# nikvaessen/w2v2-speaker

Hardware: AMD Instinct MI355X
Metric: utterances/sec (w2v2-base + mean+std + AAM-softmax training step, 3 s clips) (higher is better)
Workload: dtype f16; 1 GPU; wav2vec2-base + AAM-softmax(5994), mean+std pooling, 3 s synthetic audio, bs=66 per GPU, CNN frozen, fwd+bwd+all-reduce+Adam (BASELINE configs[1]); global_batch=66, samples_per_utt=48000, parallelism=dp1, regularisation=True

## Files before the change

### include/w2v2_hip.h

```cpp
#ifndef W2V2_HIP_H
#define W2V2_HIP_H

#include <stddef.h>
#include <stdint.h>

#ifdef __cplusplus
extern "C" {
#endif

#define W2V2_F32 0
#define W2V2_BF16 1
#define W2V2_F16 2

int w2v2_version(void);
const char* w2v2_last_error(void);

typedef struct {
  const void* ptr;
  int64_t ld;
  int64_t seg_len, seg_stride;
  int64_t stride0, stride1;
  int32_t trans;
  int32_t _pad;
} w2v2_operand;
// ... 25 lines not shown
  const float* row_scale;
  const float* col_scale;
  float alpha;
  int32_t split_k;
  int32_t accumulate;
  int32_t _pad;
  int32_t k_ext, n_ext_from;
  int64_t b_lo_offset;
} w2v2_gemm_desc;

int w2v2_gemm(const w2v2_gemm_desc* d, void* stream);
int w2v2_gemm_timed(const w2v2_gemm_desc* d, void* stream, int slot);
int w2v2_timer_read(int first_slot, int n, float* ms_out);
int w2v2_gemm_kernel_of(const w2v2_gemm_desc* d);
int w2v2_tune_gemm_kernel(int family);
int w2v2_tune_gemm_debug(int bits);
int w2v2_tune_gemm_f32_tile(int tile);
int w2v2_tune_gemm_ring_debug(int bits);
int w2v2_gemm_f32_last_kernel(void);

typedef struct {
  const void* dY; int64_t ld_dy;
  const void* X;  int64_t ld_x;
  float* dW;      int64_t ld_dw;
  float* dbias;
  int32_t n_out, n_in;
} w2v2_wgrad_problem;
int w2v2_wgrad_grouped(const w2v2_wgrad_problem* problems, int n, int tokens, int tokens_padded,
                       int dtype , void* stream);
int w2v2_wgrad_kernel_of(const w2v2_wgrad_problem* problems, int n);
// ... 358 lines not shown
```

### w2v2_speaker_amd/_lib.py

```python
from __future__ import annotations

import ctypes as C
import os

from . import _build

F32, BF16, F16 = 0, 1, 2
EPI_NONE, EPI_BIAS, EPI_BIAS_GELU, EPI_GELU_BWD, EPI_ADD, EPI_SCALE_RC, EPI_BIAS_GELU_GRAD, EPI_MUL = range(8)
OPTIM_ADAM, OPTIM_SGD = 0, 1

c_i32, c_i64, c_u64, c_f32, c_f64, c_vp = C.c_int32, C.c_int64, C.c_uint64, C.c_float, C.c_double, C.c_void_p


class Operand(C.Structure):
    _fields_ = [("ptr", c_vp), ("ld", c_i64), ("seg_len", c_i64), ("seg_stride", c_i64),
                ("stride0", c_i64), ("stride1", c_i64), ("trans", c_i32), ("_pad", c_i32)]


class GemmDesc(C.Structure):
    _fields_ = [("M", c_i32), ("N", c_i32), ("K", c_i32), ("batch", c_i32), ("batch_inner", c_i32),
                ("dtype_ab", c_i32), ("dtype_c", c_i32), ("epilogue", c_i32),
                ("A", Operand), ("B", Operand),
                ("C", c_vp), ("ldc", c_i64), ("c_stride0", c_i64), ("c_stride1", c_i64),
                ("aux", c_vp), ("ldaux", c_i64), ("aux_stride0", c_i64), ("aux_stride1", c_i64),
# ... 7 lines not shown


class WgradProblem(C.Structure):
    _fields_ = [("dY", c_vp), ("ld_dy", c_i64), ("X", c_vp), ("ld_x", c_i64), ("dW", c_vp), ("ld_dw", c_i64),
                ("dbias", c_vp), ("n_out", c_i32), ("n_in", c_i32)]


_SIGS = {
    "w2v2_version": (c_i32, []),
    "w2v2_last_error": (C.c_char_p, []),
    "w2v2_gemm": (c_i32, [C.POINTER(GemmDesc), c_vp]),
    "w2v2_gemm_kernel_of": (c_i32, [c_vp]),
    "w2v2_gemm_timed": (c_i32, [C.POINTER(GemmDesc), c_vp, c_i32]),
    "w2v2_timer_read": (c_i32, [c_i32, c_i32, c_vp]),
    "w2v2_tune_gemm_kernel": (c_i32, [c_i32]),
    "w2v2_tune_gemm_debug": (c_i32, [c_i32]),
    "w2v2_tune_gemm_f32_tile": (c_i32, [c_i32]),
    "w2v2_tune_gemm_ring_debug": (c_i32, [c_i32]),
    "w2v2_gemm_f32_last_kernel": (c_i32, []),
    "w2v2_zero_ranges": (c_i32, [c_vp, c_vp, c_i32, c_i32, c_vp]),
    "w2v2_mean": (c_i32, [c_vp, c_vp, c_i32, c_vp]),
    "w2v2_wgrad_grouped": (c_i32, [C.POINTER(WgradProblem), c_i32, c_i32, c_i32, c_i32, c_vp]),
    "w2v2_wgrad_kernel_of": (c_i32, [C.POINTER(WgradProblem), c_i32]),
    "w2v2_tune_wgrad_kernel": (c_i32, [c_i32]),
    "w2v2_conv0_workspace_floats": (c_i32, [c_i32, c_i32, c_i32, c_i32]),
    "w2v2_conv0_stats": (c_i32, [c_vp, c_vp, c_vp, c_vp, c_i32, c_i32, c_i32, c_i32, c_i32, c_f32, c_vp]),
    "w2v2_conv0_stats_mfma": (c_i32, [c_vp, c_vp, c_vp, c_vp, c_i32, c_i32, c_i32, c_i32, c_i32, c_f32, c_vp]),
    "w2v2_conv0_stats_len": (c_i32, [c_vp, c_vp, c_vp, c_vp, c_vp, c_i32, c_i32, c_i32, c_i32, c_i32, c_f32, c_vp]),
    "w2v2_conv0_stats_mfma_len": (c_i32, [c_vp, c_vp, c_vp, c_vp, c_vp, c_i32, c_i32, c_i32, c_i32, c_i32, c_f32,
                                          c_vp]),
# ... 210 lines not shown
```

### w2v2_speaker_amd/csrc/common.h

```cpp
#pragma once
#include <hip/hip_runtime.h>
#include <hip/hip_ext.h>
#include <stdint.h>
#include <stdio.h>
#include <math.h>
#include <type_traits>
#include <utility>

#include "../../include/w2v2_hip.h"

extern thread_local char g_w2v2_err[512];
#define W2V2_FAIL(...)                                   \
  do {                                                   \
    snprintf(g_w2v2_err, sizeof(g_w2v2_err), __VA_ARGS__); \
    return -1;                                           \
  } while (0)
#define W2V2_CHECK_LAUNCH(name)                                                       \
  do {                                                                                \
    hipError_t e__ = hipGetLastError();                                               \
    if (e__ != hipSuccess) W2V2_FAIL("%s: launch failed: %s", name, hipGetErrorString(e__)); \
  } while (0)
#define W2V2_REQUIRE(cond, ...) \
  do {                          \
    if (!(cond)) W2V2_FAIL(__VA_ARGS__); \
// ... 29 lines not shown
    }
  }
  hipLaunchKernelGGL(KERNEL, grid, block, lds, st, args...);
  return 0;
}

struct W2v2Switches {
  bool no_glds;
  bool glds3;
  bool tile256;
  bool persistent;
  int g3n;
  bool defer;
  bool wt_stores;
  bool late_dma;
  int reserve_cus;
  bool f32_no_dma;
  bool wgrad_ring;
  bool wgrad_ring4;
  bool wgrad_phased;
};
const W2v2Switches& w2v2_switches();
int w2v2_device_cus();

__device__ __forceinline__ void w2v2_dma16(const void* src, uint32_t lds_addr) {
  asm volatile("s_mov_b32 m0, %0\n\ts_nop 0\n\tglobal_load_lds_dwordx4 %1, off" ::"s"(lds_addr), "v"(src) : "memory", "m0");
}
__device__ __forceinline__ void w2v2_dma16(const void* src, void* lds) {
  w2v2_dma16(src, __builtin_amdgcn_readfirstlane((uint32_t)(uintptr_t)(__attribute__((address_space(3))) char*)lds));
}
// ... 376 lines not shown
```

### w2v2_speaker_amd/csrc/gemm.hip

```cpp
#include "gemm_common.h"

template <int R, bool TRANS>
struct Stager {
  static constexpr int NV = TRANS ? 4 : (R / 32);
  uint4 v[NV];

  __device__ __forceinline__ void load(const OpDev& o, const bf16_t* __restrict__ base, int r0,
                                       int rbound, int k0, int kend, int tid,
                                       const int64_t* __restrict__ rowoff) {
    if constexpr (!TRANS) {
#pragma unroll
      for (int j = 0; j < NV; ++j) {
        const int c = tid + 256 * j;
        const int row = c >> 3, kc = c & 7;
        const int k = k0 + kc * 8;
        uint4 val = make_uint4(0, 0, 0, 0);
        if (r0 + row < rbound && k < kend) {
          const bf16_t* p = base + rowoff[j] + k;
          if (o.vec_ok && k + 8 <= kend) {
            val = *reinterpret_cast<const uint4*>(p);
          } else {
            bf16_t t[8];
#pragma unroll
            for (int e = 0; e < 8; ++e) t[e] = (k + e < kend) ? p[e] : (bf16_t)0;
// ... 264 lines not shown
}

const W2v2Switches& w2v2_switches() {
  static const W2v2Switches sw = [] {
    W2v2Switches s;
    auto env_int = [](const char* name, int dflt) { const char* e = getenv(name); return e ? atoi(e) : dflt; };
    auto env_on = [](const char* name, bool dflt) { const char* e = getenv(name); return e ? e[0] != '0' : dflt; };
    s.no_glds = getenv("W2V2_NO_GLDS") != nullptr;
    s.glds3 = getenv("W2V2_NO_GLDS3") == nullptr;
    s.tile256 = getenv("W2V2_NO_GEMM_PH") == nullptr;
    s.persistent = getenv("W2V2_G3_NONPERSISTENT") == nullptr;
    s.g3n = env_int("W2V2_G3N", 512);
    s.defer = getenv("W2V2_NO_DEFER") == nullptr;
    s.wt_stores = env_on("W2V2_EPI_WT", true);
    s.late_dma = env_on("W2V2_PH_LATE", false);
    s.reserve_cus = env_int("W2V2_RESERVE_CUS", 0);
    s.f32_no_dma = env_on("W2V2_F32_NO_DMA", false);
    s.wgrad_ring = getenv("W2V2_WGRAD_V1") == nullptr;
    s.wgrad_ring4 = getenv("W2V2_NO_WGRAD4") == nullptr;
    s.wgrad_phased = getenv("W2V2_NO_WGRAD_PH") == nullptr;
    return s;
  }();
  return sw;
}

int w2v2_device_cus() {
  static const int ncu = [] {
    int dev = 0, v = 0;
    (void)hipGetDevice(&dev);
    return (hipDeviceGetAttribute(&v, hipDeviceAttributeMultiprocessorCount, dev) == hipSuccess && v > 0) ? v : 256;
  }();
  return ncu;
}
int w2v2_gemm_device_cus() {
  const int ncu = w2v2_device_cus(), r = w2v2_switches().reserve_cus;
  return (r > 0 && r < ncu) ? ncu - r : ncu;
}

static int g_w2v2_force = 0;
extern "C" int w2v2_tune_gemm_kernel(int family) {
  const int old = g_w2v2_force;
  if (family == 0 || family == 1 || family == 2 || family == 4) g_w2v2_force = family;
  return old;
}

struct GemmRoute {
  int family;
  bool narrow;
  dim3 grid;
  int f32_rows;
};

static bool aligned16(const void* p) { return (reinterpret_cast<uintptr_t>(p) & 15) == 0; }

static int gemm_route(const w2v2_gemm_desc* d, int force, GemmArgs& a, GemmRoute& r) {
  W2V2_REQUIRE(d != nullptr, "w2v2_gemm: null descriptor");
  W2V2_REQUIRE(d->M > 0 && d->N > 0 && d->K >= 0 && d->batch > 0, "w2v2_gemm: bad shape M=%d N=%d K=%d batch=%d",
               d->M, d->N, d->K, d->batch);
  W2V2_REQUIRE(d->A.ptr && d->B.ptr && d->C, "w2v2_gemm: null operand");
  W2V2_REQUIRE(d->dtype_ab == W2V2_F32 || d->dtype_ab == W2V2_BF16 || d->dtype_ab == W2V2_F16,
               "w2v2_gemm: bad dtype_ab %d", d->dtype_ab);
  W2V2_REQUIRE(d->dtype_c == W2V2_F32 || d->dtype_c == d->dtype_ab, "w2v2_gemm: dtype_c %d must be f32 or dtype_ab (%d)",
               d->dtype_c, d->dtype_ab);
  W2V2_REQUIRE(d->epilogue >= 0 && d->epilogue <= W2V2_EPI_MUL, "w2v2_gemm: bad epilogue %d", d->epilogue);
  const int split = d->split_k > 1 ? d->split_k : 1;
  const int atomic = (split > 1 || d->accumulate) ? 1 : 0;
  if (atomic) {
    W2V2_REQUIRE(d->dtype_c == W2V2_F32, "w2v2_gemm: split_k/accumulate need an f32 C");
    W2V2_REQUIRE(d->epilogue == W2V2_EPI_NONE || (split == 1) || d->epilogue == W2V2_EPI_BIAS,
                 "w2v2_gemm: split_k supports EPI_NONE/EPI_BIAS only");
// ... 25 lines not shown
  a.C = d->C; a.ldc = d->ldc; a.c_s0 = d->c_stride0; a.c_s1 = d->c_stride1;
  a.aux = d->aux; a.ldaux = d->ldaux; a.aux_s0 = d->aux_stride0; a.aux_s1 = d->aux_stride1;
  a.bias = d->bias; a.bias_s1 = d->bias_stride1;
  a.row_scale = d->row_scale; a.col_scale = d->col_scale;
  a.alpha = d->alpha;
  a.k_ext = d->k_ext; a.n_ext_from = d->n_ext_from; a.b_lo_off = d->b_lo_offset;
  a.defer_ok = 0;
  a.wt_stores = 1;
  a.late_dma = 0;
  a.xcd_tiles = 0;
  a.dbg_bits = 0;
  const int cal = d->dtype_c == W2V2_F32 ? 4 : 8;
  a.c_vec_ok = aligned16(d->C) && (d->ldc % cal == 0) && (d->c_stride0 % cal == 0) && (d->c_stride1 % cal == 0);
  a.aux_vec_ok = d->aux && aligned16(d->aux) && (d->ldaux % cal == 0) && (d->aux_stride0 % cal == 0) &&
                 (d->aux_stride1 % cal == 0);
  r.family = 0; r.narrow = false; r.grid = dim3(1); r.f32_rows = 0;

  const int bk = f32 ? 32 : 64;
  a.k_per_split = (int)(cdiv(cdiv(d->K, split), bk) * bk);
  if (a.k_per_split == 0) a.k_per_split = bk;
  if (f32) {
    r.f32_rows = w2v2_gemm_f32_dma_rows(a, d->M, d->N, d->K, split, d->batch);
    r.family = r.f32_rows > 0 ? 10 : 9;
    return 0;
  }

  const W2v2Switches& sw = w2v2_switches();
  const int64_t ncu = w2v2_gemm_device_cus();
  const bool glds = !a.A.trans && !a.B.trans && a.A.vec_ok && a.B.vec_ok && (d->K % 64 == 0) && d->K >= 64 && !sw.no_glds;
  r.narrow = d->N <= 64 || (glds && cdiv(d->M, 128) * cdiv(d->N, 128) * split * d->batch * 2 <= ncu);
  a.tiles_m = (int)cdiv(d->M, 128); a.tiles_n = (int)cdiv(d->N, r.narrow ? 64 : 128);
// ... 11 lines not shown
    phased = force == 4 && phased_ok;
  } else {
    ring = ring_ok && (d->k_ext != 0 || (d->N >= sw.g3n && d->M >= 1024 && sw.glds3));
    phased = false;
    if (ring && phased_ok && d->N >= 512 && sw.tile256) {
      const int64_t t4 = cdiv(d->M, 256) * cdiv(d->N, 256), t3 = cdiv(d->M, 256) * cdiv(d->N, 128);
      const double fill4 = (double)t4 / (double)(cdiv(t4, ncu) * ncu), fill3 = (double)t3 / (double)(cdiv(t3, ncu) * ncu);
      phased = fill4 * 1.25 >= fill3 && t4 * 2 >= ncu && (double)d->N / (double)(cdiv(d->N, 256) * 256) >= 0.9;
    }
  }
  if (d->k_ext != 0)
    W2V2_REQUIRE(ring && d->k_ext == d->K && d->n_ext_from >= 0 && d->n_ext_from % 128 == 0 && d->b_lo_offset % 8 == 0,
                 "w2v2_gemm: two-term weights (k_ext) need k_ext == K, n_ext_from %% 128 == 0 and K-contiguous 16-byte "
                 "aligned operands with K %% 64 == 0 (M=%d N=%d K=%d)", d->M, d->N, d->K);
  r.family = phased ? 4 : ring ? 2 : glds ? 1 : 3;
  a.wt_stores = sw.wt_stores;
  a.late_dma = sw.late_dma;
  if (r.family == 2)
    a.defer_ok = sw.defer && d->dtype_c != W2V2_F32 && lines_ok(a) && (d->N % 128 == 0) &&
                 d->epilogue != W2V2_EPI_BIAS_GELU && d->epilogue != W2V2_EPI_BIAS_GELU_GRAD;
  return 0;
}

extern "C" int w2v2_gemm_kernel_of(const w2v2_gemm_desc* d) {
  GemmArgs a;
  GemmRoute r;
  return gemm_route(d, g_w2v2_force, a, r) != 0 ? -1 : r.family;
}

template <typename TE, int FM, int FN, typename TC>
static int launch_glds(const GemmArgs& a, dim3 grid, hipStream_t st) {
  constexpr size_t lds = (size_t)2 * (32 * FM + 32 * FN) * 64 * sizeof(bf16_t);
  return w2v2_launch_lds<&gemm16_dma_128_kernel<TE, FM, FN, TC>>("gemm16_dma_128_kernel", grid, dim3(256), lds, st, a);
}

template <typename TE, int FM, int FN, typename TC>
static int launch_regstage(const GemmArgs& a, dim3 grid, hipStream_t st) {
  constexpr size_t lds = (size_t)2 * (32 * FM + 32 * FN) * 64 * sizeof(bf16_t);
#define W2V2_LAUNCH(TA_, TB_) \
  return w2v2_launch_lds<&gemm16_regstage_kernel<TE, FM, FN, TA_, TB_, TC>>("gemm16_regstage_kernel", grid, dim3(256), lds, st, a)
  if (!a.A.trans && !a.B.trans) W2V2_LAUNCH(false, false);
  else if (!a.A.trans && a.B.trans) W2V2_LAUNCH(false, true);
  else if (a.A.trans && !a.B.trans) W2V2_LAUNCH(true, false);
  else W2V2_LAUNCH(true, true);
#undef W2V2_LAUNCH
}

template <typename TE, typename TC>
static int launch_128(const GemmArgs& a, const GemmRoute& r, hipStream_t st) {
  if (r.family == 1) return r.narrow ? launch_glds<TE, 4, 2, TC>(a, r.grid, st) : launch_glds<TE, 4, 4, TC>(a, r.grid, st);
  return r.narrow ? launch_regstage<TE, 4, 2, TC>(a, r.grid, st) : launch_regstage<TE, 4, 4, TC>(a, r.grid, st);
}

extern "C" int w2v2_gemm(const w2v2_gemm_desc* d, void* stream) {
  GemmArgs a;
  GemmRoute r;
  if (gemm_route(d, g_w2v2_force, a, r) != 0) return -1;
  hipStream_t st = as_stream(stream);
  const bool c32 = d->dtype_c == W2V2_F32;
  int rc;
  switch (r.family) {
    case 4: rc = w2v2_launch_phased_256x256(a, d->dtype_ab, d->dtype_c, d->M, d->N, d->batch, st); break;
    case 2: rc = w2v2_launch_ring_256x128(a, d->dtype_ab, d->dtype_c, d->M, d->N, d->batch, w2v2_switches().persistent, st); break;
    case 9: case 10: rc = w2v2_launch_gemm_f32(a, d->M, d->N, d->K, a.split_k, d->batch, r.f32_rows, st); break;
    default:
      if (d->dtype_ab == W2V2_BF16) rc = c32 ? launch_128<bf16_t, float>(a, r, st) : launch_128<bf16_t, bf16_t>(a, r, st);
      else rc = c32 ? launch_128<f16_t, float>(a, r, st) : launch_128<f16_t, f16_t>(a, r, st);
      break;
  }
  if (rc != 0) return rc;
  W2V2_CHECK_LAUNCH("w2v2_gemm");
  return 0;
}

#include <vector>
W2v2PendingTimer& w2v2_pending_timer() {
  static thread_local W2v2PendingTimer t = {nullptr, nullptr, false};
// ... 32 lines not shown
```

### w2v2_speaker_amd/csrc/gemm_common.h

```cpp
#pragma once
#include "common.h"
#include <hip/hip_ext.h>
#include <type_traits>
#include <stdlib.h>

struct OpDev {
  const void* ptr;
  int64_t ld, seg_len, seg_stride;
  int trans;
  int vec_ok;
};

struct GemmArgs {
  int M, N, K;
  int epilogue, split_k, atomic;
  int tiles_m, tiles_n;
  int k_per_split;
  OpDev A, B;
  int64_t a_s0, a_s1, b_s0, b_s1;
  int batch_inner;
  void* C;
  int64_t ldc, c_s0, c_s1;
  void* aux;
  int64_t ldaux, aux_s0, aux_s1;
// ... 205 lines not shown

__device__ __forceinline__ void load_col8(const GemmArgs& g, const float* __restrict__ bias, int n, float (&cv)[8]) {
  const float* src = (g.epilogue == W2V2_EPI_SCALE_RC) ? g.col_scale : bias;
#pragma unroll
  for (int e = 0; e < 8; ++e) cv[e] = 0.f;
  if (src == nullptr || n >= g.N) return;
  if (n + 8 <= g.N && ((reinterpret_cast<uintptr_t>(src + n) & 15) == 0)) {
    const float4 a = *reinterpret_cast<const float4*>(src + n), b = *reinterpret_cast<const float4*>(src + n + 4);
    cv[0] = a.x; cv[1] = a.y; cv[2] = a.z; cv[3] = a.w; cv[4] = b.x; cv[5] = b.y; cv[6] = b.z; cv[7] = b.w;
  } else {
#pragma unroll
    for (int e = 0; e < 8; ++e) if (n + e < g.N) cv[e] = src[n + e];
  }
}

template <typename TC, int EPI, int FM, int I0, bool DEFER = false, int NR = 4>
__device__ __forceinline__ void epilogue_direct4(const GemmArgs& g, TC* __restrict__ Cz, TC* __restrict__ auxz,
                                                 f32x4 (&acc)[FM][4], int m, int n, const float (&cv0)[8],
                                                 const float (&cv1)[8], uint4 (&pend)[8]) {
  float ax[NR][16];
  if constexpr (EPI == W2V2_EPI_GELU_BWD || EPI == W2V2_EPI_ADD || EPI == W2V2_EPI_MUL) {
#pragma unroll
    for (int i = 0; i < NR; ++i) {
      const int mi = m + 16 * (I0 + i);
#pragma unroll
      for (int e = 0; e < 16; ++e) ax[i][e] = 0.f;
      if (mi < g.M) {
        const TC* ap = auxz + (int64_t)mi * g.ldaux + n;
#pragma unroll
        for (int h = 0; h < 2; ++h) {
          if (n + 8 * h + 8 <= g.N && g.aux_vec_ok) {
            Vec8<TC> t;
            t.load(ap + 8 * h);
#pragma unroll
            for (int e = 0; e < 8; ++e) ax[i][8 * h + e] = t.v[e];
          } else {
#pragma unroll
            for (int e = 0; e < 8; ++e) if (n + 8 * h + e < g.N) ax[i][8 * h + e] = to_f32<TC>(ap[8 * h + e]);
          }
        }
      }
    }
  }
#pragma unroll
  for (int i = 0; i < NR; ++i) {
    const int mi = m + 16 * (I0 + i);
    if (mi >= g.M) continue;
#pragma unroll
    for (int h = 0; h < 2; ++h) {
      if (n + 8 * h >= g.N) continue;
      float v[8];
#pragma unroll
      for (int e = 0; e < 8; ++e) v[e] = acc[I0 + i][2 * h + (e >> 2)][e & 3];
      float a8[8];
#pragma unroll
      for (int e = 0; e < 8; ++e) a8[e] = (EPI == W2V2_EPI_GELU_BWD || EPI == W2V2_EPI_ADD || EPI == W2V2_EPI_MUL) ? ax[i][8 * h + e] : 0.f;
      if constexpr (DEFER && FM == 4)
        epilogue_row8_impl<TC, EPI, true>(g, Cz, auxz, mi, n + 8 * h, v, h ? cv1 : cv0, a8, true, &pend[i * 2 + h]);
      else
        epilogue_row8_impl<TC, EPI>(g, Cz, auxz, mi, n + 8 * h, v, h ? cv1 : cv0, a8, true);
    }
  }
}
template <typename TC, int EPI, int FM, int NR = 4>
__device__ __forceinline__ void epilogue_direct(const GemmArgs& g, TC* __restrict__ Cz, TC* __restrict__ auxz,
                                                f32x4 (&acc)[FM][4], int m, int n, const float (&cv0)[8],
                                                const float (&cv1)[8]) {
  if (n >= g.N) return;
  uint4 unused[8];
  if constexpr (NR == 4) {
    epilogue_direct4<TC, EPI, FM, 0>(g, Cz, auxz, acc, m, n, cv0, cv1, unused);
    if constexpr (FM > 4) epilogue_direct4<TC, EPI, FM, 4>(g, Cz, auxz, acc, m, n, cv0, cv1, unused);
  } else {
    static_assert(NR == 2 && FM == 8, "two-row batches are wired for the 128-row wave tiles");
    epilogue_direct4<TC, EPI, FM, 0, false, 2>(g, Cz, auxz, acc, m, n, cv0, cv1, unused);
    epilogue_direct4<TC, EPI, FM, 2, false, 2>(g, Cz, auxz, acc, m, n, cv0, cv1, unused);
    epilogue_direct4<TC, EPI, FM, 4, false, 2>(g, Cz, auxz, acc, m, n, cv0, cv1, unused);
    epilogue_direct4<TC, EPI, FM, 6, false, 2>(g, Cz, auxz, acc, m, n, cv0, cv1, unused);
  }
}

__host__ __device__ __forceinline__ bool lines_ok(const GemmArgs& g) {
  return g.c_vec_ok && !g.atomic && (g.N & 63) == 0 && (g.aux == nullptr || g.aux_vec_ok);
}

template <typename TC, int EPI, int FM, bool DEFER = false>
__device__ __forceinline__ void epilogue_lines(const GemmArgs& g, TC* __restrict__ Cz, TC* __restrict__ auxz,
                                               f32x4 (&acc)[FM][4], int mw, int nc, int lane, const float (&cv0)[8],
                                               const float (&cv1)[8], uint4* __restrict__ pend) {
  static_assert(sizeof(TC) == 2, "16-bit outputs only");
  constexpr bool READS_AUX = EPI == W2V2_EPI_GELU_BWD || EPI == W2V2_EPI_ADD || EPI == W2V2_EPI_MUL;
  constexpr bool WRITES_AUX = EPI == W2V2_EPI_BIAS_GELU || EPI == W2V2_EPI_BIAS_GELU_GRAD;
  if constexpr (!DEFER) {
    if (nc >= g.N) return;
  }
  const bool wt = g.wt_stores != 0;
  auto st16 = [wt](TC* p, uint4 v) {
    if (wt) store16_wt(p, v); else *reinterpret_cast<uint4*>(p) = v;
  };
  const int c = lane & 15;
  const bool lo = c < 8;
  const int ra = mw + (c & 7);
  const int ncs = nc + (lo ? 0 : 8);
  const int mo = mw + c;
#pragma unroll
  for (int i0 = 0; i0 < FM; i0 += 4) {
    uint4 la[4], lb[4];
    if constexpr (READS_AUX) {
#pragma unroll
      for (int i = 0; i < 4; ++i) {
        const int r = ra + 16 * (i0 + i);
        la[i] = lb[i] = make_uint4(0, 0, 0, 0);
        if (r < g.M) la[i] = *reinterpret_cast<const uint4*>(auxz + (int64_t)r * g.ldaux + ncs);
        if (r + 8 < g.M) lb[i] = *reinterpret_cast<const uint4*>(auxz + (int64_t)(r + 8) * g.ldaux + ncs);
      }
    }
#pragma unroll
    for (int i = 0; i < 4; ++i) {
      float ax[16];
      if constexpr (READS_AUX) {
        uint4 a0, a1;
        lines_to_halves(lo, la[i], lb[i], a0, a1);
        unpack8<TC>(a0, ax);
        unpack8<TC>(a1, ax + 8);
      }
      float rs = 1.0f;
      if constexpr (EPI == W2V2_EPI_SCALE_RC) rs = (mo + 16 * (i0 + i) < g.M) ? g.row_scale[mo + 16 * (i0 + i)] : 0.f;
      float v[16], pre[16];
#pragma unroll
      for (int e = 0; e < 16; ++e) {
        float x = acc[i0 + i][e >> 2][e & 3] * g.alpha;
        const float cve = e < 8 ? cv0[e] : cv1[e - 8];
        if constexpr (EPI == W2V2_EPI_BIAS) x += cve;
// ... 116 lines not shown
__device__ __forceinline__ void ring_tile_srcs(const GemmArgs& g, const bf16_t* Ab, const bf16_t* Bb, int m0, int n0,
                                               int wave, int lane, const bf16_t** ap, const bf16_t** bp) {
  const int c8 = lane & 7, r8 = lane >> 3;
  int ca[4], cb[2];
#pragma unroll
  for (int j = 0; j < 4; ++j) ca[j] = (c8 ^ swz((wave * 4 + j) * 8 + r8)) << 3;
#pragma unroll
  for (int j = 0; j < 2; ++j) cb[j] = (c8 ^ swz_b((wave * 2 + j) * 8 + r8)) << 3;
  tile_ptrs<4>(g.A, Ab, m0, 256, g.M, wave * 32 + r8, 8, ca, ap);
  tile_ptrs<2>(g.B, Bb, n0, 128, g.N, wave * 16 + r8, 8, cb, bp);
}

int w2v2_gemm_device_cus();
int w2v2_launch_ring_256x128(const GemmArgs& a, int dtype_ab, int dtype_c, int M, int N, int batch, bool persistent,
                             hipStream_t st);
int w2v2_launch_phased_256x256(const GemmArgs& a, int dtype_ab, int dtype_c, int M, int N, int batch, hipStream_t st);
int w2v2_launch_gemm_f32(GemmArgs a, int M, int N, int K, int split, int batch, int dma_rows, hipStream_t st);
int w2v2_gemm_f32_dma_rows(const GemmArgs& a, int M, int N, int K, int split, int batch);
int w2v2_launch_gemm_f32_dma(const GemmArgs& a, int M, int N, int split, int batch, int fi, int nst, hipStream_t st);
bool w2v2_gemm_f32_dma_has_dbg(const GemmArgs& a, int fi);
```

### w2v2_speaker_amd/csrc/gemm_phased.hip

```cpp
#include "gemm_common.h"

template <typename TE, typename TC, int DBG = 0>
__global__ __launch_bounds__(512) void gemm16_phased_256x256_kernel(const GemmArgs g) {
  constexpr int BM = 256, BN = 256, BK = 64, FM = 8, FN = 4;
  constexpr int BUF = (BM + BN) * BK;
  extern __shared__ __attribute__((aligned(16))) char smem_raw[];
  bf16_t* smem = reinterpret_cast<bf16_t*>(smem_raw);

  const int tid = threadIdx.x;
  const int lane = tid & 63;
  const int wave = __builtin_amdgcn_readfirstlane(tid >> 6);
  const int wr = wave >> 2, wc = wave & 3;
  const int ntile = g.tiles_m * g.tiles_n;
  const int G = gridDim.x;
  const int z = blockIdx.z;
  const int z0 = z / g.batch_inner, z1 = z - z0 * g.batch_inner;
  const int nk = g.K >> 6;
  const bf16_t* Ab = reinterpret_cast<const bf16_t*>(g.A.ptr) + z0 * g.a_s0 + z1 * g.a_s1;
  const bf16_t* Bb = reinterpret_cast<const bf16_t*>(g.B.ptr) + z0 * g.b_s0 + z1 * g.b_s1;
  const int c8 = lane & 7, r8 = lane >> 3;
  const int frow = lane & 15, fk = lane >> 4;
  const int sw = swz(frow);
  const int la0 = (wr * 128 + frow) * 64 + ((fk ^ sw) << 3);
  const int la1 = (wr * 128 + frow) * 64 + (((4 + fk) ^ sw) << 3);
  const int brow = (frow >> 2) * 16 + (frow & 3);
  const int lb0 = BM * 64 + (wc * 64 + brow) * 64 + ((fk ^ sw) << 3);
  const int lb1 = BM * 64 + (wc * 64 + brow) * 64 + (((4 + fk) ^ sw) << 3);
  auto piece_row = [&](int q, int j) -> int {
    const int p = wave * 2 + j;
    if (q == 0) return (p < 8 ? p * 8 : 128 + (p - 8) * 8);
    if (q == 3) return (p < 8 ? p * 8 : 128 + (p - 8) * 8) + 64;
    return p * 16 + (q == 2 ? 8 : 0);
  };

#pragma unroll 1
  for (int t0 = 0; t0 < ntile; t0 += G) {
    const int nchunk = min(G, ntile - t0);
    if ((int)blockIdx.x >= nchunk) break;
    const int tile = t0 + xcd_remap(blockIdx.x, nchunk);
    const int tm = tile / g.tiles_n, tn = tile - tm * g.tiles_n;
    const int m0 = tm * BM, n0 = tn * BN;
    int soff[4][2];
// ... 2 lines not shown
      const bool isa = q == 0 || q == 3;
      int col[2];
      const bf16_t* ptr[2];
#pragma unroll
      for (int j = 0; j < 2; ++j) {
        const int row = piece_row(q, j) + r8;
        col[j] = (c8 ^ (isa ? swz(row) : swz_b(row))) << 3;
      }
      if (isa) tile_ptrs<2>(g.A, Ab, m0, BM, g.M, piece_row(q, 0) + r8, 8, col, ptr);
      else tile_ptrs<2>(g.B, Bb, n0, BN, g.N, piece_row(q, 0) + r8, 16, col, ptr);
#pragma unroll
      for (int j = 0; j < 2; ++j) soff[q][j] = (int)(ptr[j] - (isa ? Ab : Bb));
    }
    auto issue = [&](int q, int kt) {
      const bool isa = q == 0 || q == 3;
      bf16_t* base = smem + (kt & 1) * BUF + (isa ? 0 : BM * 64);
#pragma unroll
      for (int j = 0; j < 2; ++j)
        w2v2_dma16(((isa ? Ab : Bb) + (soff[q][j] + kt * 64)), (base + piece_row(q, j) * 64));
    };
    f32x4 acc[FM][FN];
#pragma unroll
    for (int i = 0; i < FM; ++i)
#pragma unroll
      for (int j = 0; j < FN; ++j) acc[i][j] = f32x4{0.f, 0.f, 0.f, 0.f};

    issue(0, 0); issue(1, 0); issue(2, 0); issue(3, 0);
    if (nk > 1) { issue(0, 1); issue(1, 1); }
    w2v2_vmcnt0_visible();
    __builtin_amdgcn_s_barrier();
    if (wr == 1) __builtin_amdgcn_s_barrier();
// ... 4 lines not shown
    if constexpr (NO_READ) {
#pragma unroll
      for (int j = 0; j < 2; ++j)
#pragma unroll
        for (int kk = 0; kk < 2; ++kk) {
          b0[j][kk] = *reinterpret_cast<const frag8_t*>(smem + (kk ? lb1 : lb0) + j * 4 * 64);
          b1[j][kk] = *reinterpret_cast<const frag8_t*>(smem + (kk ? lb1 : lb0) + (2 + j) * 4 * 64);
        }
#pragma unroll
      for (int i = 0; i < 4; ++i)
#pragma unroll
        for (int kk = 0; kk < 2; ++kk) af[i][kk] = *reinterpret_cast<const frag8_t*>(smem + (kk ? la1 : la0) + i * 16 * 64);
    }
    auto issue1 = [&](int q, int kt, int j) {
      const bool isa = q == 0 || q == 3;
      bf16_t* base = smem + (kt & 1) * BUF + (isa ? 0 : BM * 64);
      w2v2_dma16(((isa ? Ab : Bb) + (soff[q][j] + kt * 64)), (base + piece_row(q, j) * 64));
    };
#define W2V2_PH_MFMA(io_, jo_, bfr_, doq_, q_, kq_)                                                       \
      _Pragma("unroll") for (int kk = 0; kk < 2; ++kk) {                                                   \
        _Pragma("unroll") for (int i = 0; i < 4; ++i) {                                                    \
          if constexpr (!NO_MFMA) {                                                                        \
            _Pragma("unroll") for (int j = 0; j < 2; ++j)                                                  \
              acc[io_ + i][jo_ + j] = mfma16<TE>(bfr_[j][kk], af[i][kk], acc[io_ + i][jo_ + j]);          \
          }                                                                                                \
          if constexpr (LATE == 2 && !NO_DMA) {                                                            \
            if (i == 1 && (doq_)) {                                                                        \
              __builtin_amdgcn_sched_barrier(0);                                                           \
              issue1(q_, kq_, kk);                                                                         \
              __builtin_amdgcn_sched_barrier(0);                                                           \
            }                                                                                              \
          }                                                                                                \
          if constexpr (LATE == 1 && !NO_DMA) {                                                            \
            if (kk == 0 && i == 3 && (doq_)) {                                                             \
              __builtin_amdgcn_sched_barrier(0);                                                           \
              issue1(q_, kq_, 1);                                                                          \
              __builtin_amdgcn_sched_barrier(0);                                                           \
            }                                                                                              \
          }                                                                                                \
// ... 5 lines not shown
      const bool more1 = kt + 1 < nk, more2 = kt + 2 < nk;
      if constexpr (!NO_READ) {
#pragma unroll
        for (int j = 0; j < 2; ++j) {
          b0[j][0] = *reinterpret_cast<const frag8_t*>(bufp + lb0 + j * 4 * 64);
          b0[j][1] = *reinterpret_cast<const frag8_t*>(bufp + lb1 + j * 4 * 64);
        }
        __builtin_amdgcn_sched_barrier(0);
#pragma unroll
        for (int i = 0; i < 4; ++i) {
          af[i][0] = *reinterpret_cast<const frag8_t*>(bufp + la0 + i * 16 * 64);
          af[i][1] = *reinterpret_cast<const frag8_t*>(bufp + la1 + i * 16 * 64);
        }
      }
      if constexpr (!NO_DMA) { if (more1) { if constexpr (LATE == 0) issue(2, kt + 1); else if constexpr (LATE == 1) issue1(2, kt + 1, 0); } }
      if constexpr (!NO_DMA) wait_pieces(2 + (more1 ? 6 - LATE : 0));
      __builtin_amdgcn_s_barrier();
      asm volatile("s_waitcnt lgkmcnt(0)" ::: "memory");
      __builtin_amdgcn_sched_barrier(0);
      __builtin_amdgcn_s_setprio(1);
      W2V2_PH_MFMA(0, 0, b0, more1, 2, kt + 1)
      __builtin_amdgcn_s_setprio(0);
      __builtin_amdgcn_s_barrier();
      if constexpr (!NO_READ) {
#pragma unroll
        for (int j = 0; j < 2; ++j) {
          b1[j][0] = *reinterpret_cast<const frag8_t*>(bufp + lb0 + (2 + j) * 4 * 64);
          b1[j][1] = *reinterpret_cast<const frag8_t*>(bufp + lb1 + (2 + j) * 4 * 64);
        }
      }
      if constexpr (!NO_DMA) { if (more1) { if constexpr (LATE == 0) issue(3, kt + 1); else if constexpr (LATE == 1) issue1(3, kt + 1, 0); } }
      if constexpr (!NO_DMA) wait_pieces(more1 ? 8 - LATE : 0);
      __builtin_amdgcn_s_barrier();
      asm volatile("s_waitcnt lgkmcnt(0)" ::: "memory");
      __builtin_amdgcn_sched_barrier(0);
      __builtin_amdgcn_s_setprio(1);
      W2V2_PH_MFMA(0, 2, b1, more1, 3, kt + 1)
      __builtin_amdgcn_s_setprio(0);
      __builtin_amdgcn_s_barrier();
      if constexpr (!NO_READ) {
#pragma unroll
        for (int i = 0; i < 4; ++i) {
          af[i][0] = *reinterpret_cast<const frag8_t*>(bufp + la0 + (4 + i) * 16 * 64);
          af[i][1] = *reinterpret_cast<const frag8_t*>(bufp + la1 + (4 + i) * 16 * 64);
        }
      }
      if constexpr (!NO_DMA) { if (more2) { if constexpr (LATE == 0) issue(0, kt + 2); else if constexpr (LATE == 1) issue1(0, kt + 2, 0); } }
      __builtin_amdgcn_s_barrier();
      asm volatile("s_waitcnt lgkmcnt(0)" ::: "memory");
      __builtin_amdgcn_sched_barrier(0);
      __builtin_amdgcn_s_setprio(1);
      W2V2_PH_MFMA(4, 2, b1, more2, 0, kt + 2)
      __builtin_amdgcn_s_setprio(0);
      __builtin_amdgcn_s_barrier();
      if constexpr (!NO_DMA) { if (more2) { if constexpr (LATE == 0) issue(1, kt + 2); else if constexpr (LATE == 1) issue1(1, kt + 2, 0); } }
      if constexpr (!NO_DMA) { if (more1) wait_pieces(4 + (more2 ? 4 - LATE : 0)); }
      __builtin_amdgcn_s_barrier();
      __builtin_amdgcn_sched_barrier(0);
      __builtin_amdgcn_s_setprio(1);
      W2V2_PH_MFMA(4, 0, b0, more2, 1, kt + 2)
      __builtin_amdgcn_s_setprio(0);
      __builtin_amdgcn_s_barrier();
    }
#undef W2V2_PH_MFMA
    if (wr == 0) __builtin_amdgcn_s_barrier();

    TC* Cz = reinterpret_cast<TC*>(g.C) + z0 * g.c_s0 + z1 * g.c_s1;
    TC* auxz = g.aux ? reinterpret_cast<TC*>(g.aux) + z0 * g.aux_s0 + z1 * g.aux_s1 : nullptr;
    const float* bias = g.bias ? g.bias + z1 * g.bias_s1 : nullptr;
    int nc = n0 + wc * 64 + fk * 16, mr = m0 + wr * 128 + frow;
    asm volatile("" : "+v"(nc), "+v"(mr));
    if constexpr ((DBG & 8) != 0) { if (g.M > 0) continue; }
    float cv0[8], cv1[8];
    load_col8(g, bias, nc, cv0);
    load_col8(g, bias, nc + 8, cv1);
    if constexpr (sizeof(TC) == 2) {
      W2V2_EPI_DISPATCH((epilogue_lines<TC, EPI, FM>(g, Cz, auxz, acc, mr - frow, nc, lane, cv0, cv1, nullptr)));
    } else {
      W2V2_EPI_DISPATCH((epilogue_direct<TC, EPI, FM, 2>(g, Cz, auxz, acc, mr, nc, cv0, cv1)));
    }
  }
}

static int g_ph_dbg = 0;
extern "C" int w2v2_tune_gemm_debug(int bits) {
  const int old = g_ph_dbg;
  g_ph_dbg = bits;
  return old;
}

template <typename TE, typename TC, int DBG = 0>
static int launch_ph(GemmArgs a, int M, int N, int batch, hipStream_t st) {
  constexpr size_t lds = (size_t)2 * (256 + 256) * 64 * sizeof(bf16_t);
  a.tiles_m = (int)cdiv(M, 256);
  a.tiles_n = (int)cdiv(N, 256);
  const int tiles = a.tiles_m * a.tiles_n;
  const int ncu = w2v2_gemm_device_cus();
  dim3 grid(tiles < ncu ? tiles : ncu, 1, batch);
  return w2v2_launch_lds<&gemm16_phased_256x256_kernel<TE, TC, DBG>, true>("gemm16_phased_256x256_kernel", grid, dim3(512), lds, st, a);
}
template <typename TE, typename TC>
static int launch_ph_dbg(GemmArgs a, int M, int N, int batch, hipStream_t st) {
  if (g_ph_dbg & 192) a.wt_stores = (g_ph_dbg & 128) ? 1 : 0;
  const int variant = g_ph_dbg & 63;
  if (variant == 0 && a.late_dma) return launch_ph<TE, TC, 32>(a, M, N, batch, st);
  if constexpr (std::is_same<TE, f16_t>::value && std::is_same<TC, f16_t>::value) {
    switch (variant) {
      case 1: return launch_ph<TE, TC, 1>(a, M, N, batch, st);
      case 2: return launch_ph<TE, TC, 2>(a, M, N, batch, st);
      case 4: return launch_ph<TE, TC, 4>(a, M, N, batch, st);
      case 8: return launch_ph<TE, TC, 8>(a, M, N, batch, st);
      case 9: return launch_ph<TE, TC, 9>(a, M, N, batch, st);
      case 11: return launch_ph<TE, TC, 11>(a, M, N, batch, st);
      case 13: return launch_ph<TE, TC, 13>(a, M, N, batch, st);
      case 16: return launch_ph<TE, TC, 16>(a, M, N, batch, st);
      case 24: return launch_ph<TE, TC, 24>(a, M, N, batch, st);
      case 48: return launch_ph<TE, TC, 0>(a, M, N, batch, st);
      case 40: return launch_ph<TE, TC, 40>(a, M, N, batch, st);
      default: break;
    }
  }
  return launch_ph<TE, TC>(a, M, N, batch, st);
}
int w2v2_launch_phased_256x256(const GemmArgs& a, int dtype_ab, int dtype_c, int M, int N, int batch, hipStream_t st) {
  if (dtype_ab == W2V2_BF16)
    return dtype_c == W2V2_F32 ? launch_ph_dbg<bf16_t, float>(a, M, N, batch, st) : launch_ph_dbg<bf16_t, bf16_t>(a, M, N, batch, st);
  return dtype_c == W2V2_F32 ? launch_ph_dbg<f16_t, float>(a, M, N, batch, st) : launch_ph_dbg<f16_t, f16_t>(a, M, N, batch, st);
}
```

Baseline: 6475 utterances/sec.

## Add 240-row tile variant to phased GEMM to balance waves across CUs

```diff
diff --git a/include/w2v2_hip.h b/include/w2v2_hip.h
--- a/include/w2v2_hip.h
+++ b/include/w2v2_hip.h
@@ -63,6 +63,9 @@
 int w2v2_timer_read(int first_slot, int n, float* ms_out);
 int w2v2_gemm_kernel_of(const w2v2_gemm_desc* d);
 int w2v2_tune_gemm_kernel(int family);
+int w2v2_gemm_tile_rows(int64_t M, int64_t tiles_n, int64_t tiles_n2, int64_t batch, int64_t G);
+int w2v2_gemm_rows_of(const w2v2_gemm_desc* d);
+int w2v2_tune_gemm_rows(int rows);
 int w2v2_tune_gemm_debug(int bits);
 int w2v2_tune_gemm_f32_tile(int tile);
 int w2v2_tune_gemm_ring_debug(int bits);
diff --git a/w2v2_speaker_amd/_lib.py b/w2v2_speaker_amd/_lib.py
--- a/w2v2_speaker_amd/_lib.py
+++ b/w2v2_speaker_amd/_lib.py
@@ -45,6 +45,9 @@
     "w2v2_gemm_timed": (c_i32, [C.POINTER(GemmDesc), c_vp, c_i32]),
     "w2v2_timer_read": (c_i32, [c_i32, c_i32, c_vp]),
     "w2v2_tune_gemm_kernel": (c_i32, [c_i32]),
+    "w2v2_gemm_tile_rows": (c_i32, [c_i64, c_i64, c_i64, c_i64, c_i64]),
+    "w2v2_gemm_rows_of": (c_i32, [c_vp]),
+    "w2v2_tune_gemm_rows": (c_i32, [c_i32]),
     "w2v2_tune_gemm_debug": (c_i32, [c_i32]),
     "w2v2_tune_gemm_f32_tile": (c_i32, [c_i32]),
     "w2v2_tune_gemm_ring_debug": (c_i32, [c_i32]),
diff --git a/w2v2_speaker_amd/csrc/common.h b/w2v2_speaker_amd/csrc/common.h
--- a/w2v2_speaker_amd/csrc/common.h
+++ b/w2v2_speaker_amd/csrc/common.h
@@ -67,6 +67,7 @@
   bool defer;
   bool wt_stores;
   bool late_dma;
+  bool rows240;
   int reserve_cus;
   bool f32_no_dma;
   bool wgrad_ring;
diff --git a/w2v2_speaker_amd/csrc/gemm.hip b/w2v2_speaker_amd/csrc/gemm.hip
--- a/w2v2_speaker_amd/csrc/gemm.hip
+++ b/w2v2_speaker_amd/csrc/gemm.hip
@@ -302,6 +302,7 @@
     s.defer = getenv("W2V2_NO_DEFER") == nullptr;
     s.wt_stores = env_on("W2V2_EPI_WT", true);
     s.late_dma = env_on("W2V2_PH_LATE", false);
+    s.rows240 = env_on("W2V2_ROWS240", true);
     s.reserve_cus = env_int("W2V2_RESERVE_CUS", 0);
     s.f32_no_dma = env_on("W2V2_F32_NO_DMA", false);
     s.wgrad_ring = getenv("W2V2_WGRAD_V1") == nullptr;
@@ -332,16 +333,30 @@
   return old;
 }
 
+static int g_w2v2_pin_rows = 0;
+extern "C" int w2v2_tune_gemm_rows(int rows) {
+  const int old = g_w2v2_pin_rows;
+  if (rows == 0 || rows == 256) g_w2v2_pin_rows = rows;
+  return old;
+}
+
+extern "C" int w2v2_gemm_tile_rows(int64_t M, int64_t tiles_n, int64_t tiles_n2, int64_t batch, int64_t G) {
+  if (M <= 0 || tiles_n <= 0 || batch <= 0 || G <= 0) return 256;
+  auto cost = [&](int64_t bm) { return cdiv(cdiv(M, bm) * (tiles_n + tiles_n2) * batch, G) * bm; };
+  return cost(240) < cost(256) ? 240 : 256;
+}
+
 struct GemmRoute {
   int family;
   bool narrow;
   dim3 grid;
   int f32_rows;
+  int rows;
 };
 
 static bool aligned16(const void* p) { return (reinterpret_cast<uintptr_t>(p) & 15) == 0; }
 
-static int gemm_route(const w2v2_gemm_desc* d, int force, GemmArgs& a, GemmRoute& r) {
+static int gemm_route(const w2v2_gemm_desc* d, int force, int pin_rows, GemmArgs& a, GemmRoute& r) {
   W2V2_REQUIRE(d != nullptr, "w2v2_gemm: null descriptor");
   W2V2_REQUIRE(d->M > 0 && d->N > 0 && d->K >= 0 && d->batch > 0, "w2v2_gemm: bad shape M=%d N=%d K=%d batch=%d",
                d->M, d->N, d->K, d->batch);
@@ -397,7 +412,7 @@
   a.c_vec_ok = aligned16(d->C) && (d->ldc % cal == 0) && (d->c_stride0 % cal == 0) && (d->c_stride1 % cal == 0);
   a.aux_vec_ok = d->aux && aligned16(d->aux) && (d->ldaux % cal == 0) && (d->aux_stride0 % cal == 0) &&
                  (d->aux_stride1 % cal == 0);
-  r.family = 0; r.narrow = false; r.grid = dim3(1); r.f32_rows = 0;
+  r.family = 0; r.narrow = false; r.grid = dim3(1); r.f32_rows = 0; r.rows = 256;
 
   const int bk = f32 ? 32 : 64;
   a.k_per_split = (int)(cdiv(cdiv(d->K, split), bk) * bk);
@@ -439,6 +454,7 @@
                  "w2v2_gemm: two-term weights (k_ext) need k_ext == K, n_ext_from %% 128 == 0 and K-contiguous 16-byte "
                  "aligned operands with K %% 64 == 0 (M=%d N=%d K=%d)", d->M, d->N, d->K);
   r.family = phased ? 4 : ring ? 2 : glds ? 1 : 3;
+  if (r.family == 4 && sw.rows240 && pin_rows != 256) r.rows = w2v2_gemm_tile_rows(d->M, cdiv(d->N, 256), 0, d->batch, ncu);
   a.wt_stores = sw.wt_stores;
   a.late_dma = sw.late_dma;
   if (r.family == 2)
@@ -450,7 +466,7 @@
 extern "C" int w2v2_gemm_kernel_of(const w2v2_gemm_desc* d) {
   GemmArgs a;
   GemmRoute r;
-  return gemm_route(d, g_w2v2_force, a, r) != 0 ? -1 : r.family;
+  return gemm_route(d, g_w2v2_force, g_w2v2_pin_rows, a, r) != 0 ? -1 : r.family;
 }
 
 template <typename TE, int FM, int FN, typename TC>
@@ -477,15 +493,22 @@
   return r.narrow ? launch_regstage<TE, 4, 2, TC>(a, r.grid, st) : launch_regstage<TE, 4, 4, TC>(a, r.grid, st);
 }
 
+extern "C" int w2v2_gemm_rows_of(const w2v2_gemm_desc* d) {
+  GemmArgs a;
+  GemmRoute r;
+  if (gemm_route(d, g_w2v2_force, g_w2v2_pin_rows, a, r) != 0) return -1;
+  return (r.family == 2 || r.family == 4) ? r.rows : 128;
+}
+
 extern "C" int w2v2_gemm(const w2v2_gemm_desc* d, void* stream) {
   GemmArgs a;
   GemmRoute r;
-  if (gemm_route(d, g_w2v2_force, a, r) != 0) return -1;
+  if (gemm_route(d, g_w2v2_force, g_w2v2_pin_rows, a, r) != 0) return -1;
   hipStream_t st = as_stream(stream);
   const bool c32 = d->dtype_c == W2V2_F32;
   int rc;
   switch (r.family) {
-    case 4: rc = w2v2_launch_phased_256x256(a, d->dtype_ab, d->dtype_c, d->M, d->N, d->batch, st); break;
+    case 4: rc = w2v2_launch_phased_256x256(a, d->dtype_ab, d->dtype_c, d->M, d->N, d->batch, r.rows, st); break;
     case 2: rc = w2v2_launch_ring_256x128(a, d->dtype_ab, d->dtype_c, d->M, d->N, d->batch, w2v2_switches().persistent, st); break;
     case 9: case 10: rc = w2v2_launch_gemm_f32(a, d->M, d->N, d->K, a.split_k, d->batch, r.f32_rows, st); break;
     default:
diff --git a/w2v2_speaker_amd/csrc/gemm_common.h b/w2v2_speaker_amd/csrc/gemm_common.h
--- a/w2v2_speaker_amd/csrc/gemm_common.h
+++ b/w2v2_speaker_amd/csrc/gemm_common.h
@@ -243,10 +243,10 @@
   }
 }
 
-template <typename TC, int EPI, int FM, int I0, bool DEFER = false, int NR = 4>
+template <typename TC, int EPI, int FM, int I0, bool DEFER = false, int NR = 4, bool SHORT = false>
 __device__ __forceinline__ void epilogue_direct4(const GemmArgs& g, TC* __restrict__ Cz, TC* __restrict__ auxz,
                                                  f32x4 (&acc)[FM][4], int m, int n, const float (&cv0)[8],
-                                                 const float (&cv1)[8], uint4 (&pend)[8]) {
+                                                 const float (&cv1)[8], uint4 (&pend)[8], int nfrag = FM) {
   float ax[NR][16];
   if constexpr (EPI == W2V2_EPI_GELU_BWD || EPI == W2V2_EPI_ADD || EPI == W2V2_EPI_MUL) {
 #pragma unroll
@@ -254,7 +254,7 @@
       const int mi = m + 16 * (I0 + i);
 #pragma unroll
       for (int e = 0; e < 16; ++e) ax[i][e] = 0.f;
-      if (mi < g.M) {
+      if (mi < g.M && (!SHORT || I0 + i < nfrag)) {
         const TC* ap = auxz + (int64_t)mi * g.ldaux + n;
 #pragma unroll
         for (int h = 0; h < 2; ++h) {
@@ -275,6 +275,7 @@
   for (int i = 0; i < NR; ++i) {
     const int mi = m + 16 * (I0 + i);
     if (mi >= g.M) continue;
+    if (SHORT && I0 + i >= nfrag) continue;
 #pragma unroll
     for (int h = 0; h < 2; ++h) {
       if (n + 8 * h >= g.N) continue;
@@ -291,21 +292,21 @@
     }
   }
 }
-template <typename TC, int EPI, int FM, int NR = 4>
+template <typename TC, int EPI, int FM, int NR = 4, bool SHORT = false>
 __device__ __forceinline__ void epilogue_direct(const GemmArgs& g, TC* __restrict__ Cz, TC* __restrict__ auxz,
                                                 f32x4 (&acc)[FM][4], int m, int n, const float (&cv0)[8],
-                                                const float (&cv1)[8]) {
+                                                const float (&cv1)[8], int nfrag = FM) {
   if (n >= g.N) return;
   uint4 unused[8];
   if constexpr (NR == 4) {
-    epilogue_direct4<TC, EPI, FM, 0>(g, Cz, auxz, acc, m, n, cv0, cv1, unused);
-    if constexpr (FM > 4) epilogue_direct4<TC, EPI, FM, 4>(g, Cz, auxz, acc, m, n, cv0, cv1, unused);
+    epilogue_direct4<TC, EPI, FM, 0, false, 4, SHORT>(g, Cz, auxz, acc, m, n, cv0, cv1, unused, nfrag);
+    if constexpr (FM > 4) epilogue_direct4<TC, EPI, FM, 4, false, 4, SHORT>(g, Cz, auxz, acc, m, n, cv0, cv1, unused, nfrag);
   } else {
     static_assert(NR == 2 && FM == 8, "two-row batches are wired for the 128-row wave tiles");
-    epilogue_direct4<TC, EPI, FM, 0, false, 2>(g, Cz, auxz, acc, m, n, cv0, cv1, unused);
-    epilogue_direct4<TC, EPI, FM, 2, false, 2>(g, Cz, auxz, acc, m, n, cv0, cv1, unused);
-    epilogue_direct4<TC, EPI, FM, 4, false, 2>(g, Cz, auxz, acc, m, n, cv0, cv1, unused);
-    epilogue_direct4<TC, EPI, FM, 6, false, 2>(g, Cz, auxz, acc, m, n, cv0, cv1, unused);
+    epilogue_direct4<TC, EPI, FM, 0, false, 2, SHORT>(g, Cz, auxz, acc, m, n, cv0, cv1, unused, nfrag);
+    epilogue_direct4<TC, EPI, FM, 2, false, 2, SHORT>(g, Cz, auxz, acc, m, n, cv0, cv1, unused, nfrag);
+    epilogue_direct4<TC, EPI, FM, 4, false, 2, SHORT>(g, Cz, auxz, acc, m, n, cv0, cv1, unused, nfrag);
+    epilogue_direct4<TC, EPI, FM, 6, false, 2, SHORT>(g, Cz, auxz, acc, m, n, cv0, cv1, unused, nfrag);
   }
 }
 
@@ -313,10 +314,10 @@
   return g.c_vec_ok && !g.atomic && (g.N & 63) == 0 && (g.aux == nullptr || g.aux_vec_ok);
 }
 
-template <typename TC, int EPI, int FM, bool DEFER = false>
+template <typename TC, int EPI, int FM, bool DEFER = false, bool SHORT = false>
 __device__ __forceinline__ void epilogue_lines(const GemmArgs& g, TC* __restrict__ Cz, TC* __restrict__ auxz,
                                                f32x4 (&acc)[FM][4], int mw, int nc, int lane, const float (&cv0)[8],
-                                               const float (&cv1)[8], uint4* __restrict__ pend) {
+                                               const float (&cv1)[8], uint4* __restrict__ pend, int nfrag = FM) {
   static_assert(sizeof(TC) == 2, "16-bit outputs only");
   constexpr bool READS_AUX = EPI == W2V2_EPI_GELU_BWD || EPI == W2V2_EPI_ADD || EPI == W2V2_EPI_MUL;
   constexpr bool WRITES_AUX = EPI == W2V2_EPI_BIAS_GELU || EPI == W2V2_EPI_BIAS_GELU_GRAD;
@@ -340,12 +341,14 @@
       for (int i = 0; i < 4; ++i) {
         const int r = ra + 16 * (i0 + i);
         la[i] = lb[i] = make_uint4(0, 0, 0, 0);
+        if (SHORT && i0 + i >= nfrag) continue;
         if (r < g.M) la[i] = *reinterpret_cast<const uint4*>(auxz + (int64_t)r * g.ldaux + ncs);
         if (r + 8 < g.M) lb[i] = *reinterpret_cast<const uint4*>(auxz + (int64_t)(r + 8) * g.ldaux + ncs);
       }
     }
 #pragma unroll
     for (int i = 0; i < 4; ++i) {
+      if (SHORT && i0 + i >= nfrag) continue;
       float ax[16];
       if constexpr (READS_AUX) {
         uint4 a0, a1;
@@ -492,7 +495,8 @@
 int w2v2_gemm_device_cus();
 int w2v2_launch_ring_256x128(const GemmArgs& a, int dtype_ab, int dtype_c, int M, int N, int batch, bool persistent,
                              hipStream_t st);
-int w2v2_launch_phased_256x256(const GemmArgs& a, int dtype_ab, int dtype_c, int M, int N, int batch, hipStream_t st);
+int w2v2_launch_phased_256x256(const GemmArgs& a, int dtype_ab, int dtype_c, int M, int N, int batch, int rows,
+                               hipStream_t st);
 int w2v2_launch_gemm_f32(GemmArgs a, int M, int N, int K, int split, int batch, int dma_rows, hipStream_t st);
 int w2v2_gemm_f32_dma_rows(const GemmArgs& a, int M, int N, int K, int split, int batch);
 int w2v2_launch_gemm_f32_dma(const GemmArgs& a, int M, int N, int split, int batch, int fi, int nst, hipStream_t st);
diff --git a/w2v2_speaker_amd/csrc/gemm_phased.hip b/w2v2_speaker_amd/csrc/gemm_phased.hip
--- a/w2v2_speaker_amd/csrc/gemm_phased.hip
+++ b/w2v2_speaker_amd/csrc/gemm_phased.hip
@@ -1,9 +1,11 @@
 #include "gemm_common.h"
 
-template <typename TE, typename TC, int DBG = 0>
+template <typename TE, typename TC, int DBG = 0, int BM = 256>
 __global__ __launch_bounds__(512) void gemm16_phased_256x256_kernel(const GemmArgs g) {
-  constexpr int BM = 256, BN = 256, BK = 64, FM = 8, FN = 4;
-  constexpr int BUF = (BM + BN) * BK;
+  static_assert(BM == 256 || BM == 240, "block tile rows");
+  constexpr int AM = 256;
+  constexpr int BN = 256, BK = 64, FM = 8, FN = 4;
+  constexpr int BUF = (AM + BN) * BK;
   extern __shared__ __attribute__((aligned(16))) char smem_raw[];
   bf16_t* smem = reinterpret_cast<bf16_t*>(smem_raw);
 
@@ -11,6 +13,8 @@
   const int lane = tid & 63;
   const int wave = __builtin_amdgcn_readfirstlane(tid >> 6);
   const int wr = wave >> 2, wc = wave & 3;
+  const int nfrag = (BM == 240 && wr == 1) ? 7 : 8, nhi = nfrag - 4;
+  const int PA1 = (BM == 240 && wave == 7) ? 0 : 2;
   const int ntile = g.tiles_m * g.tiles_n;
   const int G = gridDim.x;
   const int z = blockIdx.z;
@@ -24,8 +28,8 @@
   const int la0 = (wr * 128 + frow) * 64 + ((fk ^ sw) << 3);
   const int la1 = (wr * 128 + frow) * 64 + (((4 + fk) ^ sw) << 3);
   const int brow = (frow >> 2) * 16 + (frow & 3);
-  const int lb0 = BM * 64 + (wc * 64 + brow) * 64 + ((fk ^ sw) << 3);
-  const int lb1 = BM * 64 + (wc * 64 + brow) * 64 + (((4 + fk) ^ sw) << 3);
+  const int lb0 = AM * 64 + (wc * 64 + brow) * 64 + ((fk ^ sw) << 3);
+  const int lb1 = AM * 64 + (wc * 64 + brow) * 64 + (((4 + fk) ^ sw) << 3);
   auto piece_row = [&](int q, int j) -> int {
     const int p = wave * 2 + j;
     if (q == 0) return (p < 8 ? p * 8 : 128 + (p - 8) * 8);
@@ -58,7 +62,8 @@
     }
     auto issue = [&](int q, int kt) {
       const bool isa = q == 0 || q == 3;
-      bf16_t* base = smem + (kt & 1) * BUF + (isa ? 0 : BM * 64);
+      bf16_t* base = smem + (kt & 1) * BUF + (isa ? 0 : AM * 64);
+      if (q == 3 && PA1 == 0) return;
 #pragma unroll
       for (int j = 0; j < 2; ++j)
         w2v2_dma16(((isa ? Ab : Bb) + (soff[q][j] + kt * 64)), (base + piece_row(q, j) * 64));
@@ -93,15 +98,18 @@
     }
     auto issue1 = [&](int q, int kt, int j) {
       const bool isa = q == 0 || q == 3;
-      bf16_t* base = smem + (kt & 1) * BUF + (isa ? 0 : BM * 64);
+      bf16_t* base = smem + (kt & 1) * BUF + (isa ? 0 : AM * 64);
+      if (q == 3 && PA1 == 0) return;
       w2v2_dma16(((isa ? Ab : Bb) + (soff[q][j] + kt * 64)), (base + piece_row(q, j) * 64));
     };
 #define W2V2_PH_MFMA(io_, jo_, bfr_, doq_, q_, kq_)                                                       \
       _Pragma("unroll") for (int kk = 0; kk < 2; ++kk) {                                                   \
         _Pragma("unroll") for (int i = 0; i < 4; ++i) {                                                    \
           if constexpr (!NO_MFMA) {                                                                        \
-            _Pragma("unroll") for (int j = 0; j < 2; ++j)                                                  \
-              acc[io_ + i][jo_ + j] = mfma16<TE>(bfr_[j][kk], af[i][kk], acc[io_ + i][jo_ + j]);          \
+            if (BM == 256 || io_ == 0 || i < nhi) {                                                        \
+              _Pragma("unroll") for (int j = 0; j < 2; ++j)                                                \
+                acc[io_ + i][jo_ + j] = mfma16<TE>(bfr_[j][kk], af[i][kk], acc[io_ + i][jo_ + j]);        \
+            }                                                                                              \
           }                                                                                                \
           if constexpr (LATE == 2 && !NO_DMA) {                                                            \
             if (i == 1 && (doq_)) {                                                                        \
@@ -137,7 +145,7 @@
         }
       }
       if constexpr (!NO_DMA) { if (more1) { if constexpr (LATE == 0) issue(2, kt + 1); else if constexpr (LATE == 1) issue1(2, kt + 1, 0); } }
-      if constexpr (!NO_DMA) wait_pieces(2 + (more1 ? 6 - LATE : 0));
+      if constexpr (!NO_DMA) wait_pieces(PA1 + (more1 ? 6 - LATE : 0));
       __builtin_amdgcn_s_barrier();
       asm volatile("s_waitcnt lgkmcnt(0)" ::: "memory");
       __builtin_amdgcn_sched_barrier(0);
@@ -153,7 +161,7 @@
         }
       }
       if constexpr (!NO_DMA) { if (more1) { if constexpr (LATE == 0) issue(3, kt + 1); else if constexpr (LATE == 1) issue1(3, kt + 1, 0); } }
-      if constexpr (!NO_DMA) wait_pieces(more1 ? 8 - LATE : 0);
+      if constexpr (!NO_DMA) wait_pieces(more1 ? 6 + PA1 - LATE : 0);
       __builtin_amdgcn_s_barrier();
       asm volatile("s_waitcnt lgkmcnt(0)" ::: "memory");
       __builtin_amdgcn_sched_barrier(0);
@@ -164,8 +172,10 @@
       if constexpr (!NO_READ) {
 #pragma unroll
         for (int i = 0; i < 4; ++i) {
-          af[i][0] = *reinterpret_cast<const frag8_t*>(bufp + la0 + (4 + i) * 16 * 64);
-          af[i][1] = *reinterpret_cast<const frag8_t*>(bufp + la1 + (4 + i) * 16 * 64);
+          if (BM == 256 || i < nhi) {
+            af[i][0] = *reinterpret_cast<const frag8_t*>(bufp + la0 + (4 + i) * 16 * 64);
+            af[i][1] = *reinterpret_cast<const frag8_t*>(bufp + la1 + (4 + i) * 16 * 64);
+          }
         }
       }
       if constexpr (!NO_DMA) { if (more2) { if constexpr (LATE == 0) issue(0, kt + 2); else if constexpr (LATE == 1) issue1(0, kt + 2, 0); } }
@@ -177,7 +187,7 @@
       __builtin_amdgcn_s_setprio(0);
       __builtin_amdgcn_s_barrier();
       if constexpr (!NO_DMA) { if (more2) { if constexpr (LATE == 0) issue(1, kt + 2); else if constexpr (LATE == 1) issue1(1, kt + 2, 0); } }
-      if constexpr (!NO_DMA) { if (more1) wait_pieces(4 + (more2 ? 4 - LATE : 0)); }
+      if constexpr (!NO_DMA) { if (more1) wait_pieces(2 + PA1 + (more2 ? 4 - LATE : 0)); }
       __builtin_amdgcn_s_barrier();
       __builtin_amdgcn_sched_barrier(0);
       __builtin_amdgcn_s_setprio(1);
@@ -198,9 +208,9 @@
     load_col8(g, bias, nc, cv0);
     load_col8(g, bias, nc + 8, cv1);
     if constexpr (sizeof(TC) == 2) {
-      W2V2_EPI_DISPATCH((epilogue_lines<TC, EPI, FM>(g, Cz, auxz, acc, mr - frow, nc, lane, cv0, cv1, nullptr)));
+      W2V2_EPI_DISPATCH((epilogue_lines<TC, EPI, FM, false, BM == 240>(g, Cz, auxz, acc, mr - frow, nc, lane, cv0, cv1, nullptr, nfrag)));
     } else {
-      W2V2_EPI_DISPATCH((epilogue_direct<TC, EPI, FM, 2>(g, Cz, auxz, acc, mr, nc, cv0, cv1)));
+      W2V2_EPI_DISPATCH((epilogue_direct<TC, EPI, FM, 2, BM == 240>(g, Cz, auxz, acc, mr, nc, cv0, cv1, nfrag)));
     }
   }
 }
@@ -212,20 +222,21 @@
   return old;
 }
 
-template <typename TE, typename TC, int DBG = 0>
+template <typename TE, typename TC, int DBG = 0, int BM = 256>
 static int launch_ph(GemmArgs a, int M, int N, int batch, hipStream_t st) {
   constexpr size_t lds = (size_t)2 * (256 + 256) * 64 * sizeof(bf16_t);
-  a.tiles_m = (int)cdiv(M, 256);
+  a.tiles_m = (int)cdiv(M, BM);
   a.tiles_n = (int)cdiv(N, 256);
   const int tiles = a.tiles_m * a.tiles_n;
   const int ncu = w2v2_gemm_device_cus();
   dim3 grid(tiles < ncu ? tiles : ncu, 1, batch);
-  return w2v2_launch_lds<&gemm16_phased_256x256_kernel<TE, TC, DBG>, true>("gemm16_phased_256x256_kernel", grid, dim3(512), lds, st, a);
+  return w2v2_launch_lds<&gemm16_phased_256x256_kernel<TE, TC, DBG, BM>, true>("gemm16_phased_256x256_kernel", grid, dim3(512), lds, st, a);
 }
 template <typename TE, typename TC>
-static int launch_ph_dbg(GemmArgs a, int M, int N, int batch, hipStream_t st) {
+static int launch_ph_dbg(GemmArgs a, int M, int N, int batch, int rows, hipStream_t st) {
   if (g_ph_dbg & 192) a.wt_stores = (g_ph_dbg & 128) ? 1 : 0;
   const int variant = g_ph_dbg & 63;
+  if (variant == 0 && !a.late_dma && rows == 240) return launch_ph<TE, TC, 0, 240>(a, M, N, batch, st);
   if (variant == 0 && a.late_dma) return launch_ph<TE, TC, 32>(a, M, N, batch, st);
   if constexpr (std::is_same<TE, f16_t>::value && std::is_same<TC, f16_t>::value) {
     switch (variant) {
@@ -245,8 +256,11 @@
   }
   return launch_ph<TE, TC>(a, M, N, batch, st);
 }
-int w2v2_launch_phased_256x256(const GemmArgs& a, int dtype_ab, int dtype_c, int M, int N, int batch, hipStream_t st) {
+int w2v2_launch_phased_256x256(const GemmArgs& a, int dtype_ab, int dtype_c, int M, int N, int batch, int rows,
+                               hipStream_t st) {
   if (dtype_ab == W2V2_BF16)
-    return dtype_c == W2V2_F32 ? launch_ph_dbg<bf16_t, float>(a, M, N, batch, st) : launch_ph_dbg<bf16_t, bf16_t>(a, M, N, batch, st);
-  return dtype_c == W2V2_F32 ? launch_ph_dbg<f16_t, float>(a, M, N, batch, st) : launch_ph_dbg<f16_t, f16_t>(a, M, N, batch, st);
-}
+    return dtype_c == W2V2_F32 ? launch_ph_dbg<bf16_t, float>(a, M, N, batch, rows, st)
+                               : launch_ph_dbg<bf16_t, bf16_t>(a, M, N, batch, rows, st);
+  return dtype_c == W2V2_F32 ? launch_ph_dbg<f16_t, float>(a, M, N, batch, rows, st)
+                             : launch_ph_dbg<f16_t, f16_t>(a, M, N, batch, rows, st);
+}
```

After: 6377 utterances/sec. -1.5%, worse.
